# pascalPost/turbomesh

Hardware: AMD Instinct MI355X
Metric: nodes smoothed/sec (elliptic sweeps, 4096^2 blocks) + achieved HBM GB/s (higher is better)
Workload: dtype f64

## Files before the change

turbomesh_amd/csrc/tm_kernels.h:

```cpp
#pragma once
#include <hip/hip_runtime.h>
#include <cstdint>
#include "tm_edge_types.h"
#include <vector>

namespace tmh {

enum ApplyMode : int {
    MODE_RAW = 0,
    MODE_SCALED = 1,
    MODE_RESID = 2,
    MODE_RELAX = 3,
    MODE_DIAG_COPY = 4,
    MODE_DIAG_SUM9 = 5,
    MODE_DIAG_NOSTORE = 6,
    MODE_DIAG_NOLOAD = 7,
    MODE_DIAG_MATH = 8,
    MODE_MG_RESID = 9,
    MODE_MG_SMOOTH = 10,
    MODE_MG_FIRST2 = 11
};
enum DotMode : int {
    DOT_NONE = 0,
    DOT_AUX = 1,
// ... 82 lines not shown

hipError_t launch_edge_levels3(const FusedLevelsDev& F, const EdgeRowsDev& e1, const EdgeRowsDev& e2, const EdgeRowsDev& e3, const double2* x, double2* m,
                               double2* m2, double2* out, const double2* pq, double omega, int dot, double* partials ,
                               hipStream_t stream);
hipError_t launch_edge_rows(const EdgeRowsDev& e, const double2* in, const double2* xk, const double2* pq, const double2* aux,
                            double2* out, double omega, int mode, int dot, double* partials, hipStream_t stream, uint32_t* signal = nullptr);
hipError_t launch_apply_edge_blocks(const ApplyBlock* blocks, int n, int mode, int dot, const EdgeRowsDev& e, const double2* in, const double2* xk,
                                    const double2* pq, const double2* aux, double2* out, double* edge_partials, hipStream_t stream);
constexpr int VK_NONE = 0, VK_S = 1, VK_P = 2, VK_R = 3, VK_S2 = 4, VK_PRO = 5;
struct VirtualIn {
    int kind;
    const double2 *in, *in2, *in3, *aux;
    double2* pout;
    const double2* in4 = nullptr;
    double2* rout = nullptr;
    double2* uio = nullptr;
};
hipError_t launch_apply_virtual(const ApplyBlock* blocks, int n, const EdgeRowsDev& e, const VirtualIn& V, const double2* xk, const double2* pq, double2* out,
                                double* edge_partials, const LazyScalars& scal, hipStream_t stream, bool overlap = false);
hipError_t launch_edge_rhs(const EdgeRowsDev& e, const double2* xk, const double2* pq, double2* rhs_out, int scaled,
                           double* partials , hipStream_t stream);

hipError_t launch_queue_signal(uint32_t* counter, hipStream_t stream);
hipError_t launch_queue_wait(const uint32_t* counter, uint32_t target, uint32_t* error, hipStream_t stream, long long limit_ticks = QUEUE_WAIT_TICKS);
hipError_t launch_queue_signal_wait(uint32_t* counter, const uint32_t* other, uint32_t target, uint32_t* error, hipStream_t stream,
                                    long long limit_ticks = QUEUE_WAIT_TICKS);

hipError_t launch_assemble_interior(const double2* xk, const double2* pq, int ni, int nj, const int32_t* row_ptr ,
                                    double* vx, double* vy, hipStream_t stream);
hipError_t launch_assemble_edge(const EdgeRowsDev& e, const double2* xk, const double2* pq, const int32_t* row_ptr, double* vx, double* vy, hipStream_t stream);
hipError_t launch_csr_product(int64_t n, const int32_t* row_ptr, const int32_t* col, const double* vx, const double* vy, const double2* in, double2* out,
                              hipStream_t stream);
hipError_t launch_delay_us(double us, hipStream_t stream);

hipError_t launch_finalize(const double* partials, int nwg, double* red, hipStream_t stream);

struct KrylovScalars {
    double rho[2], rho_old[2], alpha[2], omega[2], beta[2];
    double tol2[2];
    double rr[2];
    double rr0[2];
    int32_t done[2];
    int32_t early[2];
    int32_t iters;
    int32_t _pad;
};
constexpr int VEC_BLOCK = 256;
int vec_nwg(int64_t n);
enum ScalarStep : int { STEP_INIT = 0, STEP_SIGMA = 1, STEP_SS = 2, STEP_TSTT = 3, STEP_RHO = 4, STEP_TOL = 5, STEP_SS_TSTT = 6, STEP_INIT2 = 7, STEP_A2 = 8, STEP_B2 = 9 };
hipError_t launch_scalar_update(KrylovScalars* S, const double* red, int step, hipStream_t stream, double rtol = 0.0, double atol = 0.0);
hipError_t launch_finalize_scalar(const double* partials, int nwg, double* red, KrylovScalars* S, int step, hipStream_t stream, double rtol = 0.0,
                                  double atol = 0.0);
struct LazyStep {
    int step;
    const double* partials;
    int nwg;
};
struct LazyScalars {
    const KrylovScalars* S_in = nullptr;
    KrylovScalars* S_out = nullptr;
    int nsteps = 0;
    LazyStep st[2] = {{0, nullptr, 0}, {0, nullptr, 0}};
};
inline LazyScalars plain_scalars(const KrylovScalars* S) {
    LazyScalars L;
    L.S_in = S;
    return L;
}
hipError_t launch_p_update(const LazyScalars& S, const double2* r, double2* p, const double2* v, int64_t n, int nwg, hipStream_t stream);
hipError_t launch_s_update(const LazyScalars& S, const double2* r, const double2* v, double2* s, int64_t n, int nwg, double* partials,
                           hipStream_t stream);
hipError_t launch_xr_update(const LazyScalars& S, double2* u, const double2* p_hat, const double2* s_hat, const double2* s, const double2* t, double2* r,
                            const double2* r_hat, int64_t n, int nwg, double* partials, hipStream_t stream);
hipError_t launch_xr_update_vs(const LazyScalars& S, double2* u, const double2* p, const double2* v, const double2* t, double2* r, const double2* r_hat,
                               int64_t n, int nwg, double* partials, hipStream_t stream);
constexpr int GMRES_M = 30;
struct GmresScalars {
    double H[2][(GMRES_M + 1) * GMRES_M];
    double cs[2][GMRES_M], sn[2][GMRES_M];
    double g[2][GMRES_M + 1];
    double y[2][GMRES_M];
    double tol[2], beta[2], resid[2], rr0[2], scale[2];
    double rtol_initial;
    int32_t tol_initial[2];
    int32_t cols_used[2];
    int32_t done[2];
    int32_t scale_skip[2];
    int32_t j, cycle;
    int32_t sticky;
    int32_t iters[2];
};
hipError_t launch_gm_mgs(double2* w, const double2* v_prev, const double2* v_next, const double* red_prev, GmresScalars* G, int row_prev, int64_t n,
                         double* partials, hipStream_t stream);
hipError_t launch_gm_divide(double2* dst, const double2* src, const GmresScalars* G, int64_t n, hipStream_t stream);
hipError_t launch_gm_update(double2* u, const double2* V, int64_t ld, const GmresScalars* G, int64_t n, hipStream_t stream);
hipError_t launch_gm_tol(GmresScalars* G, const double* red, double rtol, double atol, hipStream_t stream, int sticky = 0);
hipError_t launch_gm_begin(GmresScalars* G, const double* red, hipStream_t stream);
hipError_t launch_gm_column(GmresScalars* G, const double* red, hipStream_t stream);
hipError_t launch_gm_backsub(GmresScalars* G, hipStream_t stream);

hipError_t launch_residual_copyback(double2* xk, const double2* u, int64_t n, int nwg, double* partials, hipStream_t stream);
hipError_t launch_stream(int kind, double2* a, const double2* b, const double2* c, double s, int64_t n, hipStream_t stream);
hipError_t launch_gather_rows(const double2* src, const int32_t* ids, int64_t n, double2* dst, hipStream_t stream);

hipError_t launch_copy_perimeter(const double2* in, double2* out, int ni, int nj, hipStream_t stream);
hipError_t launch_perimeter_sub(const double2* in, const double2* h, double2* out, int ni, int nj, hipStream_t stream);
hipError_t launch_ring_dirichlet(double2* f, const double2* X, const double2* PQ, double2* save, int ni, int nj, hipStream_t stream);
hipError_t launch_ring_restore(double2* f, const double2* save, int ni, int nj, hipStream_t stream);

hipError_t launch_tfi_block(double2* xy, int ni, int nj, const double2* x_i_min, const double2* x_i_max, const double2* x_j_min,
                            const double2* x_j_max, const double* s1, const double* s2, const double* t1, const double* t2,
                            hipStream_t stream);
hipError_t launch_tfi_linear2d(double2* xy, int ni, int nj, const double2* e_i_min, const double2* e_i_max, const double2* e_j_min,
                               const double2* e_j_max, hipStream_t stream);

struct WhiteArgs {
    const double2* x0;
    const double2* x1;
    double2* pq0;
    double2* pq1;
    int ni0, nj0, ni1, nj1;
    int le_p0, le_p1, le_fi0, le_fi1, le_dir0;
    double ds_target, theta_target;
};
hipError_t launch_white(const WhiteArgs& w, int update, hipStream_t stream);

struct MgPair {
    int nif, njf, nic, njc;
    int ci, cj;
};
hipError_t launch_mg_inject(const double2* fine, double2* coarse, const MgPair& g, double scale_x, double scale_y, hipStream_t stream);
hipError_t launch_mg_restrict(const double2* r_fine, const double2* X_coarse, double2* f_coarse, const MgPair& g, hipStream_t stream);
hipError_t launch_mg_prolong_smooth(const ApplyBlock& a, const MgPair& g, hipStream_t stream);
struct MgPairArgs {
    const double2* in = nullptr;
    const double2* xk = nullptr;
    const double2* pq = nullptr;
    const double2* f = nullptr;
    double2* out = nullptr;
    double2* out2 = nullptr;
    const double2* coarse = nullptr;
    const double2* xc = nullptr;
    double2* fc = nullptr;
    int nic = 0, njc = 0, ci = 0, cj = 0;
    int ni = 0, nj = 0;
    double omega = 1.0;
};
bool mg_pair_supported(int ni, int nj);
bool mg_pair_restrict_supported(int ni, int nj, int ci, int cj);
hipError_t launch_mg_pair(const MgPairArgs& a, int kind, hipStream_t stream);
hipError_t launch_mg_prolong_add(const double2* e_coarse, double2* e_fine, const MgPair& g, hipStream_t stream);
hipError_t launch_mg_scale(const double2* f, double2* out, int ni, int nj, double omega, hipStream_t stream);

hipError_t launch_soa_planes(const double2* in, double* plane0, double* plane1, int ni, int nj, hipStream_t stream);

hipError_t launch_debug_white_math(const double* x, const double* y, uint64_t n, double* out_acos, double* out_atan2, hipStream_t stream);

}
```

turbomesh_amd/csrc/tm_kernels.hip:

```cpp
#include "tm_kernels.h"
#include "tm_devutil.hpp"
#include "tm_refmath.h"
#include <cstdlib>
#include <type_traits>

namespace tmh {

__device__ __forceinline__ double lane_prev(double edge, double v) {
    int2 o = __builtin_bit_cast(int2, edge), s = __builtin_bit_cast(int2, v), r;
    r.x = __builtin_amdgcn_update_dpp(o.x, s.x, 0x138 , 0xf, 0xf, false);
    r.y = __builtin_amdgcn_update_dpp(o.y, s.y, 0x138, 0xf, 0xf, false);
    return __builtin_bit_cast(double, r);
}
__device__ __forceinline__ double lane_next(double edge, double v) {
    int2 o = __builtin_bit_cast(int2, edge), s = __builtin_bit_cast(int2, v), r;
    r.x = __builtin_amdgcn_update_dpp(o.x, s.x, 0x130 , 0xf, 0xf, false);
    r.y = __builtin_amdgcn_update_dpp(o.y, s.y, 0x130, 0xf, 0xf, false);
    return __builtin_bit_cast(double, r);
}
__device__ __forceinline__ double2 lane_prev(double2 edge, double2 v) { return make_double2(lane_prev(edge.x, v.x), lane_prev(edge.y, v.y)); }
__device__ __forceinline__ double2 lane_next(double2 edge, double2 v) { return make_double2(lane_next(edge.x, v.x), lane_next(edge.y, v.y)); }

__device__ __forceinline__ double2 lane_prev0(double2 v) {
    int4 s = __builtin_bit_cast(int4, v), r;
// ... 1713 lines not shown
    double acc[MAX_PARTIALS] = {0.0, 0.0, 0.0, 0.0};
    edge_rows_wg<MODE_SCALED, DOT, VK>(e, blockIdx.x, threadIdx.x, V.in, xk, pq, V.aux, out, 0.0, acc, A);
    block_partials<EDGE_BLOCK, (VK == VK_R ? 4 : dot_columns(DOT))>(acc, partials + static_cast<size_t>(blockIdx.x) * MAX_PARTIALS);
}


hipError_t launch_edge_rows(const EdgeRowsDev& e, const double2* in, const double2* xk, const double2* pq, const double2* aux,
                            double2* out, double omega, int mode, int dot, double* partials, hipStream_t st, uint32_t* signal) {
    if (e.nrows == 0) return signal ? launch_queue_signal(signal, st) : hipSuccess;
    const dim3 grid(e.nwg), block(EDGE_BLOCK);
#define TM_EDGE(M, D)                                                                                                  \
    if (mode == M && dot == D) {                                                                                       \
        hipLaunchKernelGGL((k_edge_rows<M, D>), grid, block, 0, st, e, in, xk, pq, aux, out, omega, partials, signal); \
        return hipGetLastError();                                                                                      \
    }
    TM_EDGE(MODE_RAW, DOT_NONE)
    TM_EDGE(MODE_SCALED, DOT_NONE)
    TM_EDGE(MODE_SCALED, DOT_AUX)
    TM_EDGE(MODE_SCALED, DOT_AUX2)
    TM_EDGE(MODE_SCALED, DOT_IN)
    TM_EDGE(MODE_RESID, DOT_OUT2)
    TM_EDGE(MODE_RESID, DOT_NONE)
    TM_EDGE(MODE_RELAX, DOT_DELTA)
    TM_EDGE(MODE_RELAX, DOT_NONE)
#undef TM_EDGE
    return hipErrorInvalidValue;
}

hipError_t launch_apply_edge_blocks(const ApplyBlock* blocks, int n, int mode, int dot, const EdgeRowsDev& e, const double2* in, const double2* xk,
                                    const double2* pq, const double2* aux, double2* out, double* edge_partials, hipStream_t st) {
    if (n > APPLY_BATCH_MAX || e.nrows == 0) return hipErrorNotSupported;
    ApplyBatch B;
    B.n = 0;
    int total = 0;
    for (int k = 0; k < n; ++k) {
        const ApplyBlock& a = blocks[k];
        if (a.in == a.xk) return hipErrorNotSupported;
        if (a.ni < 3 || a.nj < 3) continue;
        const int q = B.n++;
        B.b[q] = a;
        B.RI[q] = rows_per_chunk(a.ni, a.nj, a.rows);
        B.nSG[q] = (a.nj + 255) / 256;
        B.nRC[q] = (a.ni - 2 + B.RI[q] - 1) / B.RI[q];
        B.start[q] = total;
        total += B.nSG[q] * B.nRC[q];
    }
    for (int q = B.n; q < APPLY_BATCH_MAX; ++q) B.start[q] = total;
    const dim3 grid(total + e.nwg), block(256);
    const bool has_pq = pq != nullptr;
#define TM_AE(M, D)                                                                                                                       \
    if (mode == M && dot == D) {                                                                                                          \
        if (has_pq) hipLaunchKernelGGL((k_apply_edge_batch<M, D, true>), grid, block, 0, st, B, total, e, in, xk, pq, aux, out, edge_partials);   \
        else hipLaunchKernelGGL((k_apply_edge_batch<M, D, false>), grid, block, 0, st, B, total, e, in, xk, pq, aux, out, edge_partials);         \
        return hipGetLastError();                                                                                                         \
    }
    TM_AE(MODE_SCALED, DOT_AUX)
    TM_AE(MODE_SCALED, DOT_IN)
    TM_AE(MODE_RESID, DOT_OUT2)
#undef TM_AE
    return hipErrorNotSupported;
}

hipError_t launch_apply_virtual(const ApplyBlock* blocks, int n, const EdgeRowsDev& e, const VirtualIn& V, const double2* xk, const double2* pq, double2* out,
                                double* edge_partials, const LazyScalars& scal, hipStream_t st, bool overlap) {
    if (overlap && V.kind != VK_R && V.kind != VK_S2) return hipErrorInvalidValue;
    if (e.nrows == 0 || V.kind < VK_S || V.kind > VK_S2) return hipErrorInvalidValue;
    const bool has_pq = pq != nullptr;
    const bool merged = n <= APPLY_BATCH_MAX;
    LazyScalars L = scal;
    for (int first = 0; first < n; first += APPLY_BATCH_MAX) {
        ApplyBatch B;
        B.n = 0;
        int total = 0;
        for (int k = first; k < n && B.n < APPLY_BATCH_MAX; ++k) {
            const ApplyBlock& a = blocks[k];
            if (a.ni < 3 || a.nj < 3) continue;
            const int q = B.n++;
            B.b[q] = a;
            B.RI[q] = rows_per_chunk(a.ni, a.nj, a.rows);
            B.nSG[q] = overlap ? overlap_strip_groups(a.nj) : (a.nj + 255) / 256;
            B.nRC[q] = (a.ni - 2 + B.RI[q] - 1) / B.RI[q];
            B.start[q] = total;
            total += B.nSG[q] * B.nRC[q];
        }
        for (int q = B.n; q < APPLY_BATCH_MAX; ++q) B.start[q] = total;
        const dim3 grid(merged ? total + e.nwg : total), block(256);
        if (grid.x == 0) continue;
        const int ti = merged ? total : -1;
        if (overlap) {
            if (V.kind == VK_R) {
                if (has_pq) hipLaunchKernelGGL((k_apply_vk<true, VK_R, 2, true>), grid, block, 0, st, B, ti, e, V, xk, pq, out, edge_partials, L);
                else hipLaunchKernelGGL((k_apply_vk<false, VK_R, 2, true>), grid, block, 0, st, B, ti, e, V, xk, pq, out, edge_partials, L);
            } else {
                if (has_pq) hipLaunchKernelGGL((k_apply_vk<true, VK_S2, 2, true>), grid, block, 0, st, B, ti, e, V, xk, pq, out, edge_partials, L);
                else hipLaunchKernelGGL((k_apply_vk<false, VK_S2, 2, true>), grid, block, 0, st, B, ti, e, V, xk, pq, out, edge_partials, L);
            }
        } else
#define TM_VK(PQ, K) hipLaunchKernelGGL((k_apply_vk<PQ, K, 2>), grid, block, 0, st, B, ti, e, V, xk, pq, out, edge_partials, L)
#define TM_VK1(PQ, K) hipLaunchKernelGGL((k_apply_vk<PQ, K, 1>), grid, block, 0, st, B, ti, e, V, xk, pq, out, edge_partials, L)
        if (V.kind == VK_S) {
            if (has_pq) TM_VK(true, VK_S);
            else TM_VK(false, VK_S);
        } else if (V.kind == VK_P) {
            if (has_pq) TM_VK(true, VK_P);
            else TM_VK(false, VK_P);
        } else if (V.kind == VK_R) {
            if (grid.x > 2048 || grid.x <= 256) {
                if (has_pq) TM_VK1(true, VK_R);
                else TM_VK1(false, VK_R);
            } else {
                if (has_pq) TM_VK(true, VK_R);
                else TM_VK(false, VK_R);
            }
        } else {
            if (has_pq) TM_VK(true, VK_S2);
            else TM_VK(false, VK_S2);
        }
#undef TM_VK
#undef TM_VK1
        const hipError_t rc = hipGetLastError();
        if (rc != hipSuccess) return rc;
        if (L.nsteps) {
            L.S_in = L.S_out;
            L.S_out = nullptr;
            L.nsteps = 0;
        }
    }
    if (!merged) {
        if (V.kind == VK_S) hipLaunchKernelGGL(k_edge_rows_vk<VK_S>, dim3(e.nwg), dim3(EDGE_BLOCK), 0, st, e, V, xk, pq, out, edge_partials, L.S_in);
        else if (V.kind == VK_P) hipLaunchKernelGGL(k_edge_rows_vk<VK_P>, dim3(e.nwg), dim3(EDGE_BLOCK), 0, st, e, V, xk, pq, out, edge_partials, L.S_in);
        else if (V.kind == VK_R) hipLaunchKernelGGL(k_edge_rows_vk<VK_R>, dim3(e.nwg), dim3(EDGE_BLOCK), 0, st, e, V, xk, pq, out, edge_partials, L.S_in);
        else hipLaunchKernelGGL(k_edge_rows_vk<VK_S2>, dim3(e.nwg), dim3(EDGE_BLOCK), 0, st, e, V, xk, pq, out, edge_partials, L.S_in);
        return hipGetLastError();
    }
    return hipSuccess;
}


__device__ __forceinline__ int mg_fine_of(int c, int coarsened, int nf) { return coarsened ? min(2 * c, nf - 1) : c; }

__global__ __launch_bounds__(256) void k_mg_inject(const double2* __restrict__ fine, double2* __restrict__ coarse, MgPair g, double sx, double sy) {
    const int cj = blockIdx.x * 256 + threadIdx.x;
    if (cj >= g.njc) return;
    for (int ci = blockIdx.y; ci < g.nic; ci += gridDim.y) {
        const double2 v = fine[static_cast<size_t>(mg_fine_of(ci, g.ci, g.nif)) * g.njf + mg_fine_of(cj, g.cj, g.njf)];
        coarse[static_cast<size_t>(ci) * g.njc + cj] = make_double2(sx * v.x, sy * v.y);
    }
}
hipError_t launch_mg_inject(const double2* fine, double2* coarse, const MgPair& g, double sx, double sy, hipStream_t st) {
    hipLaunchKernelGGL(k_mg_inject, dim3((g.njc + 255) / 256, std::min(g.nic, 65535)), dim3(256), 0, st, fine, coarse, g, sx, sy);
    return hipGetLastError();
}

__global__ __launch_bounds__(256) void k_mg_restrict(const double2* __restrict__ rf, const double2* __restrict__ Xc, double2* __restrict__ fc, MgPair g) {
    const int cj = blockIdx.x * 256 + threadIdx.x + 1;
    if (cj > g.njc - 2) return;
    for (int ci = blockIdx.y + 1; ci <= g.nic - 2; ci += gridDim.y) {
    const int fi = g.ci ? 2 * ci : ci, fj = g.cj ? 2 * cj : cj;
    double2 acc = make_double2(0.0, 0.0);
#pragma unroll
    for (int di = -1; di <= 1; ++di) {
        if (!g.ci && di != 0) continue;
        const double wi = g.ci ? (di == 0 ? 0.5 : 0.25) : 1.0;
#pragma unroll
        for (int dj = -1; dj <= 1; ++dj) {
            if (!g.cj && dj != 0) continue;
            const double w = wi * (g.cj ? (dj == 0 ? 0.5 : 0.25) : 1.0);
            const double2 v = rf[static_cast<size_t>(fi + di) * g.njf + (fj + dj)];
            acc.x = fma(w, v.x, acc.x);
            acc.y = fma(w, v.y, acc.y);
        }
    }
    const size_t o = static_cast<size_t>(ci) * g.njc + cj;
    const double2 xp = Xc[o + g.njc], xm = Xc[o - g.njc], xr = Xc[o + 1], xl = Xc[o - 1];
    const double dxx = xp.x - xm.x, dxy = xp.y - xm.y, dex = xr.x - xl.x, dey = xr.y - xl.y;
    const double aii = -0.5 * (fma(dxx, dxx, dxy * dxy) + fma(dex, dex, dey * dey));
    const double k = static_cast<double>((g.ci ? 4 : 1) * (g.cj ? 4 : 1)) / ((aii == 0.0) ? 1.0 : aii);
    fc[o] = make_double2(k * acc.x, k * acc.y);
    }
}
hipError_t launch_mg_restrict(const double2* rf, const double2* Xc, double2* fc, const MgPair& g, hipStream_t st) {
    if (g.nic < 3 || g.njc < 3) return hipSuccess;
    hipLaunchKernelGGL(k_mg_restrict, dim3((g.njc - 2 + 255) / 256, std::min(g.nic - 2, 65535)), dim3(256), 0, st, rf, Xc, fc, g);
    return hipGetLastError();
}

__global__ __launch_bounds__(256) void k_mg_prolong_add(const double2* __restrict__ ec, double2* __restrict__ ef, MgPair g) {
    const int j = blockIdx.x * 256 + threadIdx.x + 1;
    if (j > g.njf - 2) return;
    for (int i = blockIdx.y + 1; i <= g.nif - 2; i += gridDim.y) {
    int ci0 = i, ci1 = i, cj0 = j, cj1 = j;
    if (g.ci) {
        ci0 = i >> 1;
        ci1 = (i + 1) >> 1;
    }
    if (g.cj) {
        cj0 = j >> 1;
        cj1 = (j + 1) >> 1;
    }
    const double2 a = ec[static_cast<size_t>(ci0) * g.njc + cj0], b = ec[static_cast<size_t>(ci0) * g.njc + cj1];
    const double2 c = ec[static_cast<size_t>(ci1) * g.njc + cj0], d = ec[static_cast<size_t>(ci1) * g.njc + cj1];
    double2 e = ef[static_cast<size_t>(i) * g.njf + j];
    e.x += 0.25 * ((a.x + b.x) + (c.x + d.x));
    e.y += 0.25 * ((a.y + b.y) + (c.y + d.y));
    ef[static_cast<size_t>(i) * g.njf + j] = e;
    }
}
hipError_t launch_mg_prolong_add(const double2* ec, double2* ef, const MgPair& g, hipStream_t st) {
    if (g.nif < 3 || g.njf < 3) return hipSuccess;
    hipLaunchKernelGGL(k_mg_prolong_add, dim3((g.njf - 2 + 255) / 256, std::min(g.nif - 2, 65535)), dim3(256), 0, st, ec, ef, g);
    return hipGetLastError();
}

__global__ __launch_bounds__(256) void k_mg_scale(const double2* __restrict__ f, double2* __restrict__ out, int ni, int nj, double omega) {
    const int j = blockIdx.x * 256 + threadIdx.x;
    if (j >= nj) return;
    for (int i = blockIdx.y; i < ni; i += gridDim.y) {
        const bool interior = i >= 1 && i <= ni - 2 && j >= 1 && j <= nj - 2;
        const size_t o = static_cast<size_t>(i) * nj + j;
        const double2 v = interior ? f[o] : make_double2(0.0, 0.0);
        out[o] = make_double2(omega * v.x, omega * v.y);
    }
}
hipError_t launch_mg_scale(const double2* f, double2* out, int ni, int nj, double omega, hipStream_t st) {
    hipLaunchKernelGGL(k_mg_scale, dim3((nj + 255) / 256, std::min(ni, 65535)), dim3(256), 0, st, f, out, ni, nj, omega);
    return hipGetLastError();
}

__global__ __launch_bounds__(256) void k_soa_planes(const double2* __restrict__ in, double* __restrict__ plane0, double* __restrict__ plane1, int ni,
                                                    int nj) {
    __shared__ double2 tile[32][33];
    const int tx = threadIdx.x & 31, ty = threadIdx.x >> 5;
    const int i0 = blockIdx.y * 32, j0 = blockIdx.x * 32;
#pragma unroll
    for (int r = 0; r < 32; r += 8) {
        const int i = i0 + ty + r, j = j0 + tx;
        if (i < ni && j < nj) tile[ty + r][tx] = in[static_cast<size_t>(i) * nj + j];
    }
    __syncthreads();
#pragma unroll
    for (int r = 0; r < 32; r += 8) {
        const int j = j0 + ty + r, i = i0 + tx;
        if (i < ni && j < nj) {
            const double2 v = tile[tx][ty + r];
            const size_t o = static_cast<size_t>(j) * ni + i;
            plane0[o] = v.x;
            plane1[o] = v.y;
        }
    }
}
hipError_t launch_soa_planes(const double2* in, double* plane0, double* plane1, int ni, int nj, hipStream_t st) {
    const dim3 grid((nj + 31) / 32, (ni + 31) / 32), block(256);
    hipLaunchKernelGGL(k_soa_planes, grid, block, 0, st, in, plane0, plane1, ni, nj);
    return hipGetLastError();
}

__global__ __launch_bounds__(EDGE_BLOCK) void k_edge_rhs(EdgeRowsDev e, const double2* __restrict__ xk, const double2* __restrict__ pq,
                                                         double2* __restrict__ rhs_out, int scaled, double* partials) {
    const EdgeRun& R = e.runs[__builtin_amdgcn_readfirstlane(e.wg_run[blockIdx.x])];
    const int k = __builtin_amdgcn_readfirstlane(e.wg_k0[blockIdx.x]) + static_cast<int>(threadIdx.x);
    double acc[MAX_PARTIALS] = {0.0, 0.0, 0.0, 0.0};
    if (k < R.count) {
        const int row = R.row0 + k * R.row_stride;
        double rhs_x, rhs_y, diag_x, diag_y;
        if (R.kind == 1) {
            const double2 im1_j = xk[R.met0[0] + k * R.met_stride[0]], ip1_j = xk[R.met0[1] + k * R.met_stride[1]];
            const double2 i_jm1 = xk[R.met0[2] + k * R.met_stride[2]];
            double2 i_jp1 = xk[R.met0[3] + k * R.met_stride[3]];
            const bool periodic = R.flags & 1;
            const double per_x = R.per[0], per_y = R.per[1];
            if (periodic) {
                i_jp1.x = i_jp1.x + (-per_x);
                i_jp1.y = i_jp1.y + (-per_y);
            }
            const double2 cf = pq ? pq[row] : make_double2(0.0, 0.0);
            const double P = periodic ? cf.x : cf.y, Q = periodic ? cf.y : cf.x;
            double c[9];
            stencil_coefs<true>(im1_j, ip1_j, i_jm1, i_jp1, P, Q, c);
            diag_x = diag_y = c[S_I_J];
            const double cs = c[S_IM1_JP1] + c[S_I_JP1] + c[S_IP1_JP1];
            rhs_x = periodic ? per_x * cs : 0.0;
            rhs_y = periodic ? per_y * cs : 0.0;
        } else {
            const int self = R.self;
            diag_x = 0.0;
            diag_y = 0.0;
#pragma unroll
            for (int q = 0; q < 9; ++q)
                if (q == self) {
                    diag_x = R.cx[q];
                    diag_y = R.cy[q];
                }
            rhs_x = e.rhs[2 * (R.first + k)];
            rhs_y = e.rhs[2 * (R.first + k) + 1];
        }
        const double bx = rhs_x * ((diag_x == 0.0) ? 1.0 : 1.0 / diag_x);
        const double by = rhs_y * ((diag_y == 0.0) ? 1.0 : 1.0 / diag_y);
        if (rhs_out) rhs_out[row] = scaled ? make_double2(bx, by) : make_double2(rhs_x, rhs_y);
        acc[0] = bx * bx;
        acc[1] = by * by;
    }
    if (partials) block_partials<EDGE_BLOCK, 2>(acc, partials + static_cast<size_t>(blockIdx.x) * MAX_PARTIALS);
}
hipError_t launch_edge_rhs(const EdgeRowsDev& e, const double2* xk, const double2* pq, double2* rhs_out, int scaled, double* partials,
                           hipStream_t st) {
    if (e.nrows == 0) return hipSuccess;
    hipLaunchKernelGGL(k_edge_rhs, dim3(e.nwg), dim3(EDGE_BLOCK), 0, st, e, xk, pq, rhs_out, scaled, partials);
    return hipGetLastError();
}

__global__ __launch_bounds__(64) void k_queue_signal(uint32_t* counter) {
    if (threadIdx.x == 0) __hip_atomic_fetch_add(counter, 1u, __ATOMIC_RELEASE, __HIP_MEMORY_SCOPE_AGENT);
}
__global__ __launch_bounds__(64) void k_queue_wait(const uint32_t* counter, uint32_t target, uint32_t* error, long long limit_ticks) {
    if (threadIdx.x == 0) spin_until(counter, target, error, limit_ticks);
}
__global__ __launch_bounds__(64) void k_queue_signal_wait(uint32_t* counter, const uint32_t* other, uint32_t target, uint32_t* error, long long limit_ticks) {
    if (threadIdx.x != 0) return;
    __hip_atomic_fetch_add(counter, 1u, __ATOMIC_RELEASE, __HIP_MEMORY_SCOPE_AGENT);
    spin_until(other, target, error, limit_ticks);
}
hipError_t launch_queue_signal_wait(uint32_t* counter, const uint32_t* other, uint32_t target, uint32_t* error, hipStream_t st, long long limit_ticks) {
    hipLaunchKernelGGL(k_queue_signal_wait, dim3(1), dim3(64), 0, st, counter, other, target, error, limit_ticks);
    return hipGetLastError();
}
template <bool HAS_PQ>
__global__ __launch_bounds__(256) void k_assemble_interior(const double2* __restrict__ xk, const double2* __restrict__ pq, int ni, int nj,
                                                           const int32_t* __restrict__ row_ptr, double* __restrict__ vx, double* __restrict__ vy) {
    const int j = blockIdx.x * 256 + threadIdx.x;
    if (j < 1 || j > nj - 2) return;
    for (int i = 1 + static_cast<int>(blockIdx.y); i <= ni - 2; i += gridDim.y) {
        const size_t at = static_cast<size_t>(i) * nj + j;
        double c[9];
        const double2 cf = HAS_PQ ? pq[at] : make_double2(0.0, 0.0);
        stencil_coefs<HAS_PQ>(xk[at - nj], xk[at + nj], xk[at - 1], xk[at + 1], cf.x, cf.y, c);
        const int e = row_ptr[at];
        const double v[9] = {c[S_IM1_JM1], c[S_IM1_J], c[S_IM1_JP1], c[S_I_JM1], c[S_I_J], c[S_I_JP1], c[S_IP1_JM1], c[S_IP1_J], c[S_IP1_JP1]};
#pragma unroll
        for (int q = 0; q < 9; ++q) {
            vx[e + q] = v[q];
            vy[e + q] = v[q];
        }
    }
}
hipError_t launch_assemble_interior(const double2* xk, const double2* pq, int ni, int nj, const int32_t* row_ptr, double* vx, double* vy, hipStream_t st) {
    if (ni < 3 || nj < 3) return hipSuccess;
    const dim3 grid((nj + 255) / 256, std::min(ni - 2, 4096));
    if (pq) hipLaunchKernelGGL(k_assemble_interior<true>, grid, dim3(256), 0, st, xk, pq, ni, nj, row_ptr, vx, vy);
    else hipLaunchKernelGGL(k_assemble_interior<false>, grid, dim3(256), 0, st, xk, pq, ni, nj, row_ptr, vx, vy);
    return hipGetLastError();
}
__global__ __launch_bounds__(EDGE_BLOCK) void k_assemble_edge(EdgeRowsDev e, const double2* __restrict__ xk, const double2* __restrict__ pq,
                                                              const int32_t* __restrict__ row_ptr, double* __restrict__ vx, double* __restrict__ vy) {
    const EdgeRun& R = e.runs[__builtin_amdgcn_readfirstlane(e.wg_run[blockIdx.x])];
    const int k = __builtin_amdgcn_readfirstlane(e.wg_k0[blockIdx.x]) + static_cast<int>(threadIdx.x);
    if (k >= R.count) return;
    const int row = R.row0 + k * R.row_stride;
    const int e0 = row_ptr[row];
    if (R.kind == 1 ) {
        const double2 im1_j = xk[R.met0[0] + k * R.met_stride[0]], ip1_j = xk[R.met0[1] + k * R.met_stride[1]];
        const double2 i_jm1 = xk[R.met0[2] + k * R.met_stride[2]];
        double2 i_jp1 = xk[R.met0[3] + k * R.met_stride[3]];
        const bool periodic = R.flags & 1;
        if (periodic) {
            i_jp1.x = i_jp1.x + (-R.per[0]);
            i_jp1.y = i_jp1.y + (-R.per[1]);
        }
        const double2 cf = pq ? pq[row] : make_double2(0.0, 0.0);
        const double P = periodic ? cf.x : cf.y, Q = periodic ? cf.y : cf.x;
        double c[9];
        stencil_coefs<true>(im1_j, ip1_j, i_jm1, i_jp1, P, Q, c);
#pragma unroll
        for (int q = 0; q < 9; ++q) {
            const double ck = pick9(c, R.slot[q]);
            vx[e0 + q] = ck;
            vy[e0 + q] = ck;
        }
        return;
// ... 734 lines not shown
```

turbomesh_amd/csrc/tm_multigrid.cpp:

```cpp
#include "tm_multigrid.hpp"
#include "tm_smoother.hpp"

#include <algorithm>
#include <cmath>
#include <cstdio>
#include <cstdlib>

namespace tmh {

#define HIPCHK(x) hip_check((x), #x)

static void log_aspect_stats(const double* xy, int ni, int nj, double& mean, double& sdev) {
    mean = sdev = 0.0;
    if (!xy || ni < 3 || nj < 3) return;
    const int si = std::max(1, (ni - 2) / 64), sj = std::max(1, (nj - 2) / 64);
    double sum = 0.0, sum2 = 0.0;
    long cnt = 0;
    for (int i = 1; i < ni - 1; i += si)
        for (int j = 1; j < nj - 1; j += sj) {
            const double* c = xy + 2 * (static_cast<size_t>(i) * nj + j);
            const double ax = c[2 * nj] - c[-2 * nj], ay = c[2 * nj + 1] - c[-2 * nj + 1];
            const double bx = c[2] - c[-2], by = c[3] - c[-1];
            const double g11 = ax * ax + ay * ay, g22 = bx * bx + by * by;
            if (g11 > 0.0 && g22 > 0.0) {
                const double l = std::log(g11 / g22);
                sum += l;
                sum2 += l * l;
                cnt += 1;
            }
        }
    if (!cnt) return;
    mean = sum / static_cast<double>(cnt);
    sdev = std::sqrt(std::max(0.0, sum2 / static_cast<double>(cnt) - mean * mean));
}

double BlockMG::aspect_of(const double* xy, int ni, int nj) {
    double mean, sdev;
    log_aspect_stats(xy, ni, nj, mean, sdev);
    return std::exp(mean);
}

double BlockMG::aspect_spread_of(const double* xy, int ni, int nj) {
    double mean, sdev;
    log_aspect_stats(xy, ni, nj, mean, sdev);
    return sdev;
}

void BlockMG::build(DeviceArena& arena, int ni, int nj, bool has_pq, double aspect, bool worst_case) {
    if (nj < 3 || ni < 3) throw TmError(TM_E_UNSUPPORTED, "multigrid: a block needs at least 3 x 3 nodes");
    if (const char* e = std::getenv("TM_MG_CYCLE")) {
        int a = nu_pre, b = nu_post, c = nu_coarsest;
        double w = omega;
        if (std::sscanf(e, "%d,%d,%d,%lf", &a, &b, &c, &w) >= 2 && a >= 0 && b >= 0 && a + b >= 1 && c >= 0 && w > 0.0 && w < 2.0) {
            nu_pre = a;
            nu_post = b;
            nu_coarsest = c;
            omega = w;
        }
    }
    if (const char* e = std::getenv("TM_MG_FUSE_PROLONG")) {
        fuse_prolong = std::atoi(e) != 0;
        fuse_prolong_min = std::atoi(e) == 2 ? 0 : fuse_prolong_min;
    }
    if (const char* e = std::getenv("TM_MG_PAIR")) use_pair = std::atoi(e) != 0;
    if (const char* e = std::getenv("TM_MG_RESTRICT_FUSED")) fuse_restrict = std::atoi(e) != 0;
    L.clear();
    MgLevel l0;
    l0.ni = ni;
    l0.nj = nj;
    L.push_back(l0);
    if (worst_case) {
        const uint64_t n = static_cast<uint64_t>(ni) * nj + 64 * 256;
        for (int k = 0; k < (has_pq ? 6 : 5); ++k) (void)arena.alloc_n<double2>(n);
        return;
    }
    double ratio = aspect > 0.0 ? aspect : 1.0;
    while (L.size() < 24) {
        const MgLevel& f = L.back();
        MgLevel c;
        c.ci = f.ni >= 5;
        c.cj = f.nj >= 5;
        if (c.ci && c.cj) {
            if (ratio > 4.0) c.ci = 0;
            else if (ratio < 0.25) c.cj = 0;
        }
        if (!c.ci && !c.cj) break;
        if (c.ci && !c.cj) ratio *= 4.0;
        if (c.cj && !c.ci) ratio *= 0.25;
        c.ni = c.ci ? f.ni / 2 + 1 : f.ni;
        c.nj = c.cj ? f.nj / 2 + 1 : f.nj;
        const uint64_t n = static_cast<uint64_t>(c.ni) * c.nj;
        c.X = arena.alloc_n<double2>(n);
        if (has_pq) c.PQ = arena.alloc_n<double2>(n);
        c.f = arena.alloc_n<double2>(n);
        c.a = arena.alloc_n<double2>(n);
        c.b = arena.alloc_n<double2>(n);
        c.r = arena.alloc_n<double2>(n);
        for (double2* q : {c.f, c.a, c.b, c.r}) HIPCHK(hipMemset(q, 0, sizeof(double2) * n));
        L.push_back(c);
    }
}

MgPair BlockMG::pair(size_t fine) const {
    const MgLevel &f = L[fine], &c = L[fine + 1];
    MgPair g;
    g.nif = f.ni;
    g.njf = f.nj;
    g.nic = c.ni;
    g.njc = c.nj;
    g.ci = c.ci;
    g.cj = c.cj;
    return g;
}

void BlockMG::set_field(const double2* X0, const double2* PQ0, hipStream_t st) {
    L[0].X = const_cast<double2*>(X0);
    L[0].PQ = const_cast<double2*>(PQ0);
    for (size_t l = 0; l + 1 < L.size(); ++l) {
        const MgPair g = pair(l);
        HIPCHK(launch_mg_inject(L[l].X, L[l + 1].X, g, 1.0, 1.0, st));
        if (PQ0) HIPCHK(launch_mg_inject(L[l].PQ, L[l + 1].PQ, g, g.ci ? 2.0 : 1.0, g.cj ? 2.0 : 1.0, st));
    }
}

void BlockMG::smooth(const MgLevel& l, const double2* f, const double2* in, double2* out, hipStream_t st) const {
    ApplyBlock a;
    a.in = in;
    a.xk = l.X;
    a.pq = l.PQ;
    a.aux = f;
    a.out = out;
    a.ni = l.ni;
    a.nj = l.nj;
    a.omega = omega;
    a.partials = nullptr;
    HIPCHK(launch_apply_block(a, MODE_MG_SMOOTH, DOT_NONE, st));
}

void BlockMG::residual(const MgLevel& l, const double2* f, const double2* in, double2* out, hipStream_t st) const {
    ApplyBlock a;
    a.in = in;
    a.xk = l.X;
    a.pq = l.PQ;
    a.aux = f;
    a.out = out;
    a.ni = l.ni;
    a.nj = l.nj;
    a.omega = 0.0;
    a.partials = nullptr;
    HIPCHK(launch_apply_block(a, MODE_MG_RESID, DOT_NONE, st));
}

void BlockMG::vcycle(const double2* f0, double2* z, double2* w0, double2* w1, hipStream_t st) {
    const size_t nl = L.size();
    std::vector<double2*> cur(nl, nullptr), oth(nl, nullptr);
    std::vector<const double2*> rhs(nl, nullptr);
    const int pre_extra = nu_pre > 0 ? nu_pre - 1 : 0;
    auto pair_ok = [&](size_t l) { return use_pair && mg_pair_supported(L[l].ni, L[l].nj); };
    const bool pair_pre0 = pair_ok(0) && nu_pre == 2 && nl > 1, pair_post0 = pair_ok(0) && nu_post == 2;
    (void)pair_pre0;
    const int flips0 = (nl == 1) ? pre_extra + nu_coarsest : pre_extra + (pair_post0 ? 1 : nu_post);
    cur[0] = (flips0 % 2 == 0) ? z : w0;
    oth[0] = (flips0 % 2 == 0) ? w0 : z;
    rhs[0] = f0;
    L[0].r = w1;
    for (size_t l = 1; l < nl; ++l) {
        cur[l] = L[l].a;
        oth[l] = L[l].b;
        rhs[l] = L[l].f;
    }
    auto sweeps = [&](size_t l, int n) {
        for (int k = 0; k < n; ++k) {
            smooth(L[l], rhs[l], cur[l], oth[l], st);
            std::swap(cur[l], oth[l]);
        }
    };
    for (size_t l = 0; l < nl; ++l) {
        if (l == 0) {
            HIPCHK(launch_copy_perimeter(w1, cur[0], L[0].ni, L[0].nj, st));
            HIPCHK(launch_copy_perimeter(w1, oth[0], L[0].ni, L[0].nj, st));
        }
        if (nu_pre == 2 && l + 1 < nl && pair_ok(l)) {
            MgPairArgs a;
            a.in = rhs[l];
            a.xk = L[l].X;
            a.pq = L[l].PQ;
            a.out = oth[l];
            a.out2 = L[l].r;
            a.ni = L[l].ni;
            a.nj = L[l].nj;
            a.omega = omega;
            const MgPair g = pair(l);
            if (fuse_restrict && mg_pair_restrict_supported(a.ni, a.nj, g.ci, g.cj)) {
                a.out2 = nullptr;
                a.xc = L[l + 1].X;
                a.fc = L[l + 1].f;
                a.nic = g.nic;
                a.njc = g.njc;
                a.ci = g.ci;
                a.cj = g.cj;
                HIPCHK(launch_mg_pair(a, 1, st));
                std::swap(cur[l], oth[l]);
                continue;
            }
            HIPCHK(launch_mg_pair(a, 1, st));
            std::swap(cur[l], oth[l]);
            HIPCHK(launch_mg_restrict(L[l].r, L[l + 1].X, L[l + 1].f, g, st));
            continue;
        }
        if (nu_pre >= 2) {
            ApplyBlock a;
            a.in = rhs[l];
            a.xk = L[l].X;
            a.pq = L[l].PQ;
            a.aux = nullptr;
            a.out = oth[l];
            a.ni = L[l].ni;
            a.nj = L[l].nj;
            a.omega = omega;
            a.partials = nullptr;
            HIPCHK(launch_apply_block(a, MODE_MG_FIRST2, DOT_NONE, st));
            std::swap(cur[l], oth[l]);
            sweeps(l, pre_extra - 1);
        } else {
            HIPCHK(launch_mg_scale(rhs[l], cur[l], L[l].ni, L[l].nj, nu_pre > 0 ? omega : 0.0, st));
            sweeps(l, pre_extra);
        }
        if (l + 1 == nl) {
            sweeps(l, nu_coarsest);
            break;
        }
        residual(L[l], rhs[l], cur[l], L[l].r, st);
        HIPCHK(launch_mg_restrict(L[l].r, L[l + 1].X, L[l + 1].f, pair(l), st));
    }
    for (size_t l = nl - 1; l-- > 0;) {
        if (nu_post == 2 && pair_ok(l)) {
            MgPairArgs a;
            a.in = cur[l];
            a.xk = L[l].X;
            a.pq = L[l].PQ;
            a.f = rhs[l];
            a.out = oth[l];
            a.coarse = cur[l + 1];
            const MgPair g = pair(l);
            a.nic = g.nic;
            a.njc = g.njc;
            a.ci = g.ci;
            a.cj = g.cj;
            a.ni = L[l].ni;
            a.nj = L[l].nj;
            a.omega = omega;
            HIPCHK(launch_mg_pair(a, 0, st));
            std::swap(cur[l], oth[l]);
            continue;
        }
        if (fuse_prolong && nu_post >= 1 && static_cast<int64_t>(L[l].ni) * L[l].nj >= fuse_prolong_min) {
            ApplyBlock a;
            a.in = cur[l];
            a.in2 = cur[l + 1];
            a.xk = L[l].X;
            a.pq = L[l].PQ;
            a.aux = rhs[l];
            a.out = oth[l];
            a.ni = L[l].ni;
            a.nj = L[l].nj;
            a.omega = omega;
            a.partials = nullptr;
            HIPCHK(launch_mg_prolong_smooth(a, pair(l), st));
            std::swap(cur[l], oth[l]);
            sweeps(l, nu_post - 1);
        } else {
            HIPCHK(launch_mg_prolong_add(cur[l + 1], cur[l], pair(l), st));
            sweeps(l, nu_post);
        }
    }
    if (cur[0] != z) throw TmError(TM_E_ARG, "internal: multigrid result landed in the scratch block");
}

}
```

turbomesh_amd/csrc/tm_multigrid.hpp:

```cpp
#pragma once
#include "tm_kernels.h"
#include <vector>

namespace tmh {

class DeviceArena;

struct MgLevel {
    int ni = 0, nj = 0;
    int ci = 0, cj = 0;
    double2 *X = nullptr, *PQ = nullptr;
    double2 *f = nullptr, *a = nullptr, *b = nullptr, *r = nullptr;
};

class BlockMG {
   public:
    int nu_pre = 2, nu_post = 2, nu_coarsest = 8;
    int64_t fuse_prolong_min = 262144;
    bool fuse_prolong = true;
    double omega = 0.8;
    bool fuse_restrict = true;
    bool use_pair = true;
    void build(DeviceArena& arena, int ni, int nj, bool has_pq, double aspect, bool worst_case);
    static double aspect_of(const double* xy, int ni, int nj);
    static double aspect_spread_of(const double* xy, int ni, int nj);
    void set_field(const double2* X0, const double2* PQ0, hipStream_t stream);
    void vcycle(const double2* f, double2* z, double2* w0, double2* w1, hipStream_t stream);
    size_t nlevels() const { return L.size(); }
    const std::vector<MgLevel>& levels() const { return L; }

   private:
    std::vector<MgLevel> L;
    void smooth(const MgLevel& l, const double2* f, const double2* in, double2* out, hipStream_t st) const;
    void residual(const MgLevel& l, const double2* f, const double2* in, double2* out, hipStream_t st) const;
    MgPair pair(size_t fine) const;
};

}
```

Baseline: 448.2 billion.

## Run coarse multigrid levels in a single persistent one-block kernel

Adds a single-workgroup kernel that runs the whole coarse tail of the V-cycle (pre-smoothing, residual, restriction, coarsest sweeps, prolongation, post-smoothing) for all levels whose size is at most a threshold, using __syncthreads between phases. This replaces many tiny kernel launches on small grids, whose cost is dominated by launch latency, with one launch. In exchange those levels run on one CU only, and the ping-pong buffer parity must be worked out on the host to find the result buffer.

After: 448.0 billion, median of 3. About the same (-0.0%).

```diff
diff --git a/turbomesh_amd/csrc/tm_kernels.h b/turbomesh_amd/csrc/tm_kernels.h
--- a/turbomesh_amd/csrc/tm_kernels.h
+++ b/turbomesh_amd/csrc/tm_kernels.h
@@ -258,6 +258,21 @@
 hipError_t launch_mg_prolong_add(const double2* e_coarse, double2* e_fine, const MgPair& g, hipStream_t stream);
 hipError_t launch_mg_scale(const double2* f, double2* out, int ni, int nj, double omega, hipStream_t stream);
 
+constexpr int MG_TAIL_MAX = 24;
+struct MgTailLevel {
+    const double2 *X = nullptr, *PQ = nullptr;
+    double2 *f = nullptr, *a = nullptr, *b = nullptr, *r = nullptr;
+    int ni = 0, nj = 0, ci = 0, cj = 0;
+};
+struct MgTailArgs {
+    MgTailLevel L[MG_TAIL_MAX];
+    int n = 0;
+    int nu_pre = 2, nu_post = 2, nu_coarsest = 8;
+    double omega = 1.0;
+};
+double2* mg_tail_result(const MgTailArgs& a);
+hipError_t launch_mg_tail(const MgTailArgs& a, hipStream_t stream);
+
 hipError_t launch_soa_planes(const double2* in, double* plane0, double* plane1, int ni, int nj, hipStream_t stream);
 
 hipError_t launch_debug_white_math(const double* x, const double* y, uint64_t n, double* out_acos, double* out_atan2, hipStream_t stream);
diff --git a/turbomesh_amd/csrc/tm_kernels.hip b/turbomesh_amd/csrc/tm_kernels.hip
--- a/turbomesh_amd/csrc/tm_kernels.hip
+++ b/turbomesh_amd/csrc/tm_kernels.hip
@@ -1889,10 +1889,7 @@
     return hipGetLastError();
 }
 
-__global__ __launch_bounds__(256) void k_mg_restrict(const double2* __restrict__ rf, const double2* __restrict__ Xc, double2* __restrict__ fc, MgPair g) {
-    const int cj = blockIdx.x * 256 + threadIdx.x + 1;
-    if (cj > g.njc - 2) return;
-    for (int ci = blockIdx.y + 1; ci <= g.nic - 2; ci += gridDim.y) {
+__device__ __forceinline__ void mg_restrict_node(const double2* __restrict__ rf, const double2* __restrict__ Xc, double2* __restrict__ fc, const MgPair& g, int ci, int cj) {
     const int fi = g.ci ? 2 * ci : ci, fj = g.cj ? 2 * cj : cj;
     double2 acc = make_double2(0.0, 0.0);
 #pragma unroll
@@ -1914,7 +1911,11 @@
     const double aii = -0.5 * (fma(dxx, dxx, dxy * dxy) + fma(dex, dex, dey * dey));
     const double k = static_cast<double>((g.ci ? 4 : 1) * (g.cj ? 4 : 1)) / ((aii == 0.0) ? 1.0 : aii);
     fc[o] = make_double2(k * acc.x, k * acc.y);
-    }
+}
+__global__ __launch_bounds__(256) void k_mg_restrict(const double2* __restrict__ rf, const double2* __restrict__ Xc, double2* __restrict__ fc, MgPair g) {
+    const int cj = blockIdx.x * 256 + threadIdx.x + 1;
+    if (cj > g.njc - 2) return;
+    for (int ci = blockIdx.y + 1; ci <= g.nic - 2; ci += gridDim.y) mg_restrict_node(rf, Xc, fc, g, ci, cj);
 }
 hipError_t launch_mg_restrict(const double2* rf, const double2* Xc, double2* fc, const MgPair& g, hipStream_t st) {
     if (g.nic < 3 || g.njc < 3) return hipSuccess;
@@ -1922,10 +1923,7 @@
     return hipGetLastError();
 }
 
-__global__ __launch_bounds__(256) void k_mg_prolong_add(const double2* __restrict__ ec, double2* __restrict__ ef, MgPair g) {
-    const int j = blockIdx.x * 256 + threadIdx.x + 1;
-    if (j > g.njf - 2) return;
-    for (int i = blockIdx.y + 1; i <= g.nif - 2; i += gridDim.y) {
+__device__ __forceinline__ void mg_prolong_node(const double2* __restrict__ ec, double2* __restrict__ ef, const MgPair& g, int i, int j) {
     int ci0 = i, ci1 = i, cj0 = j, cj1 = j;
     if (g.ci) {
         ci0 = i >> 1;
@@ -1941,7 +1939,11 @@
     e.x += 0.25 * ((a.x + b.x) + (c.x + d.x));
     e.y += 0.25 * ((a.y + b.y) + (c.y + d.y));
     ef[static_cast<size_t>(i) * g.njf + j] = e;
-    }
+}
+__global__ __launch_bounds__(256) void k_mg_prolong_add(const double2* __restrict__ ec, double2* __restrict__ ef, MgPair g) {
+    const int j = blockIdx.x * 256 + threadIdx.x + 1;
+    if (j > g.njf - 2) return;
+    for (int i = blockIdx.y + 1; i <= g.nif - 2; i += gridDim.y) mg_prolong_node(ec, ef, g, i, j);
 }
 hipError_t launch_mg_prolong_add(const double2* ec, double2* ef, const MgPair& g, hipStream_t st) {
     if (g.nif < 3 || g.njf < 3) return hipSuccess;
@@ -1961,6 +1963,123 @@
 }
 hipError_t launch_mg_scale(const double2* f, double2* out, int ni, int nj, double omega, hipStream_t st) {
     hipLaunchKernelGGL(k_mg_scale, dim3((nj + 255) / 256, std::min(ni, 65535)), dim3(256), 0, st, f, out, ni, nj, omega);
+    return hipGetLastError();
+}
+
+enum { TAIL_FIRST2 = 0, TAIL_SMOOTH, TAIL_RESID };
+template <int OP, bool HAS_PQ>
+__device__ __forceinline__ void mg_tail_sweep(const MgTailLevel& L, const double2* in, double2* out, double omega, int tid, int nt) {
+    const int nj = L.nj, wj = nj - 2, n = (L.ni - 2) * wj;
+    auto row_of = [&](size_t o) {
+        const double2 l = in[o - 1], r = in[o + 1];
+        Row3 w;
+        w.c = in[o];
+        w.e = sub2(r, l);
+        w.h = add2(r, l);
+        return w;
+    };
+    for (int k = tid; k < n; k += nt) {
+        const int i = k / wj;
+        const size_t o = static_cast<size_t>(i + 1) * nj + (k - i * wj + 1);
+        const MgMetric M = mg_metric(sub2(L.X[o + nj], L.X[o - nj]), sub2(L.X[o + 1], L.X[o - 1]));
+        const Row3 c = row_of(o);
+        const double2 pq = HAS_PQ ? L.PQ[o] : make_double2(0.0, 0.0);
+        const double2 t = mg_scaled_row<HAS_PQ>(M, row_of(o - nj), c, row_of(o + nj), pq.x, pq.y);
+        double2 v;
+        if (OP == TAIL_FIRST2) {
+            v = make_double2(omega * fma(-omega, t.x, 2.0 * c.c.x), omega * fma(-omega, t.y, 2.0 * c.c.y));
+        } else {
+            const double2 res = sub2(L.f[o], t);
+            if (OP == TAIL_RESID) {
+                const double aii = -0.5 * M.D;
+                v = make_double2(aii * res.x, aii * res.y);
+            } else {
+                v = make_double2(fma(omega, res.x, c.c.x), fma(omega, res.y, c.c.y));
+            }
+        }
+        out[o] = v;
+    }
+    __syncthreads();
+}
+
+template <bool HAS_PQ>
+__global__ __launch_bounds__(1024) void k_mg_tail(MgTailArgs A) {
+    const int tid = threadIdx.x, nt = blockDim.x, nl = A.n;
+    unsigned flip = 0;
+    auto cur = [&](int l) { return ((flip >> l) & 1u) ? A.L[l].b : A.L[l].a; };
+    auto oth = [&](int l) { return ((flip >> l) & 1u) ? A.L[l].a : A.L[l].b; };
+    auto pair_of = [&](int l) {
+        MgPair g;
+        g.nif = A.L[l].ni;
+        g.njf = A.L[l].nj;
+        g.nic = A.L[l + 1].ni;
+        g.njc = A.L[l + 1].nj;
+        g.ci = A.L[l + 1].ci;
+        g.cj = A.L[l + 1].cj;
+        return g;
+    };
+    auto sweeps = [&](int l, int n) {
+        for (int k = 0; k < n; ++k) {
+            mg_tail_sweep<TAIL_SMOOTH, HAS_PQ>(A.L[l], cur(l), oth(l), A.omega, tid, nt);
+            flip ^= 1u << l;
+        }
+    };
+    for (int l = 0; l < nl; ++l) {
+        const MgTailLevel& L = A.L[l];
+        if (A.nu_pre >= 2) {
+            mg_tail_sweep<TAIL_FIRST2, HAS_PQ>(L, L.f, oth(l), A.omega, tid, nt);
+            flip ^= 1u << l;
+            sweeps(l, A.nu_pre - 2);
+        } else {
+            const double w = A.nu_pre > 0 ? A.omega : 0.0;
+            double2* e = cur(l);
+            const int wj = L.nj - 2, n = (L.ni - 2) * wj;
+            for (int k = tid; k < n; k += nt) {
+                const int i = k / wj;
+                const size_t o = static_cast<size_t>(i + 1) * L.nj + (k - i * wj + 1);
+                const double2 v = L.f[o];
+                e[o] = make_double2(w * v.x, w * v.y);
+            }
+            __syncthreads();
+        }
+        if (l + 1 == nl) {
+            sweeps(l, A.nu_coarsest);
+            break;
+        }
+        mg_tail_sweep<TAIL_RESID, HAS_PQ>(L, cur(l), L.r, 0.0, tid, nt);
+        const MgPair g = pair_of(l);
+        const int wj = g.njc - 2, n = (g.nic - 2) * wj;
+        for (int k = tid; k < n; k += nt) {
+            const int i = k / wj;
+            mg_restrict_node(L.r, A.L[l + 1].X, A.L[l + 1].f, g, i + 1, k - i * wj + 1);
+        }
+        __syncthreads();
+    }
+    for (int l = nl - 2; l >= 0; --l) {
+        const MgPair g = pair_of(l);
+        const double2* ec = cur(l + 1);
+        double2* ef = cur(l);
+        const int wj = g.njf - 2, n = (g.nif - 2) * wj;
+        for (int k = tid; k < n; k += nt) {
+            const int i = k / wj;
+            mg_prolong_node(ec, ef, g, i + 1, k - i * wj + 1);
+        }
+        __syncthreads();
+        sweeps(l, A.nu_post);
+    }
+}
+double2* mg_tail_result(const MgTailArgs& A) {
+    const int flips = std::max(A.nu_pre - 1, 0) + (A.n == 1 ? A.nu_coarsest : A.nu_post);
+    return (flips % 2 == 0) ? A.L[0].a : A.L[0].b;
+}
+hipError_t launch_mg_tail(const MgTailArgs& A, hipStream_t st) {
+    if (A.n < 1 || A.n > MG_TAIL_MAX) return hipErrorInvalidValue;
+    for (int l = 0; l < A.n; ++l)
+        if (A.L[l].ni < 3 || A.L[l].nj < 3) return hipErrorInvalidValue;
+    const int64_t nodes = static_cast<int64_t>(A.L[0].ni - 2) * (A.L[0].nj - 2);
+    const int threads = static_cast<int>(std::min<int64_t>(1024, (nodes + 63) / 64 * 64));
+    if (A.L[0].PQ) hipLaunchKernelGGL(k_mg_tail<true>, dim3(1), dim3(threads), 0, st, A);
+    else hipLaunchKernelGGL(k_mg_tail<false>, dim3(1), dim3(threads), 0, st, A);
     return hipGetLastError();
 }
 
diff --git a/turbomesh_amd/csrc/tm_multigrid.cpp b/turbomesh_amd/csrc/tm_multigrid.cpp
--- a/turbomesh_amd/csrc/tm_multigrid.cpp
+++ b/turbomesh_amd/csrc/tm_multigrid.cpp
@@ -3,6 +3,7 @@
 
 #include <algorithm>
 #include <cmath>
+#include <cstdint>
 #include <cstdio>
 #include <cstdlib>
 
@@ -64,6 +65,11 @@
     }
     if (const char* e = std::getenv("TM_MG_PAIR")) use_pair = std::atoi(e) != 0;
     if (const char* e = std::getenv("TM_MG_RESTRICT_FUSED")) fuse_restrict = std::atoi(e) != 0;
+    if (const char* e = std::getenv("TM_MG_TAIL")) {
+        tail_max_nodes = std::atoi(e) == 0 ? 0 : (std::atoi(e) == 2 ? INT64_MAX : tail_max_nodes);
+    }
+    if (const char* e = std::getenv("TM_MG_TAIL_NODES"))
+        if (tail_max_nodes > 0 && std::atoll(e) > 0) tail_max_nodes = std::atoll(e);
     L.clear();
     MgLevel l0;
     l0.ni = ni;
@@ -98,6 +104,29 @@
         c.r = arena.alloc_n<double2>(n);
         for (double2* q : {c.f, c.a, c.b, c.r}) HIPCHK(hipMemset(q, 0, sizeof(double2) * n));
         L.push_back(c);
+    }
+    tail.n = 0;
+    for (size_t l = 1; l < L.size(); ++l) {
+        if (static_cast<int64_t>(L[l].ni) * L[l].nj > tail_max_nodes || L.size() - l > static_cast<size_t>(MG_TAIL_MAX)) continue;
+        l_tail = l;
+        for (size_t k = l; k < L.size(); ++k) {
+            MgTailLevel& t = tail.L[tail.n++];
+            t.X = L[k].X;
+            t.PQ = L[k].PQ;
+            t.f = L[k].f;
+            t.a = L[k].a;
+            t.b = L[k].b;
+            t.r = L[k].r;
+            t.ni = L[k].ni;
+            t.nj = L[k].nj;
+            t.ci = L[k].ci;
+            t.cj = L[k].cj;
+        }
+        tail.nu_pre = nu_pre;
+        tail.nu_post = nu_post;
+        tail.nu_coarsest = nu_coarsest;
+        tail.omega = omega;
+        break;
     }
 }
 
@@ -175,7 +204,13 @@
             std::swap(cur[l], oth[l]);
         }
     };
+    const size_t top = tail.n > 0 ? l_tail : nl - 1;
     for (size_t l = 0; l < nl; ++l) {
+        if (tail.n > 0 && l == l_tail) {
+            HIPCHK(launch_mg_tail(tail, st));
+            cur[l] = mg_tail_result(tail);
+            break;
+        }
         if (l == 0) {
             HIPCHK(launch_copy_perimeter(w1, cur[0], L[0].ni, L[0].nj, st));
             HIPCHK(launch_copy_perimeter(w1, oth[0], L[0].ni, L[0].nj, st));
@@ -233,7 +268,7 @@
         residual(L[l], rhs[l], cur[l], L[l].r, st);
         HIPCHK(launch_mg_restrict(L[l].r, L[l + 1].X, L[l + 1].f, pair(l), st));
     }
-    for (size_t l = nl - 1; l-- > 0;) {
+    for (size_t l = top; l-- > 0;) {
         if (nu_post == 2 && pair_ok(l)) {
             MgPairArgs a;
             a.in = cur[l];
diff --git a/turbomesh_amd/csrc/tm_multigrid.hpp b/turbomesh_amd/csrc/tm_multigrid.hpp
--- a/turbomesh_amd/csrc/tm_multigrid.hpp
+++ b/turbomesh_amd/csrc/tm_multigrid.hpp
@@ -20,6 +20,7 @@
     bool fuse_prolong = true;
     double omega = 0.8;
     bool fuse_restrict = true;
+    int64_t tail_max_nodes = 1089;
     bool use_pair = true;
     void build(DeviceArena& arena, int ni, int nj, bool has_pq, double aspect, bool worst_case);
     static double aspect_of(const double* xy, int ni, int nj);
@@ -31,6 +32,8 @@
 
    private:
     std::vector<MgLevel> L;
+    MgTailArgs tail;
+    size_t l_tail = 0;
     void smooth(const MgLevel& l, const double2* f, const double2* in, double2* out, hipStream_t st) const;
     void residual(const MgLevel& l, const double2* f, const double2* in, double2* out, hipStream_t st) const;
     MgPair pair(size_t fine) const;
```
